# jchen8tw/ewn-gym

Measured on AMD Instinct MI355X. Metric: env steps/sec (whole node), 5x5 EWN, depth-3 expectiminimax opponent, higher is better.
Workload: dtype u32 bitboards (int8 boards in HBM), f64 expectation

## Files before the change

ewn_gym_amd/csrc/ewn_rollout.hpp:

```cpp
#pragma once
#include "ewn_step_d3.hpp"


#ifdef EWN_ROLLOUT_STAMPS
#define RSTAMP(i) do { unsigned long long t_; asm volatile("s_memtime %0\n\ts_waitcnt lgkmcnt(0)" : "=s"(t_) :: "memory"); st_acc[i] += t_ - st_prev; st_prev = t_; } while (0)
#else
#define RSTAMP(i) do { } while (0)
#endif

struct RollCfg {
    int N, autoreset, lane_offset, depth, agent_depth, K;
    int agent_sample;
    u32 seed_stride, W;
    double reward;
    u64 key;
};

struct RollBuf {
    int8_t *board; int8_t *dice; uint8_t *done; u32 *rng;
    const void *tables;
    const void *agent_tables;
    int8_t *t_board; int8_t *t_dice; int8_t *t_action; double *t_reward; uint8_t *t_term; uint8_t *t_trunc; uint8_t *t_info;
    uint8_t *t_rec;
    double *ret_sum; int32_t *n_steps; int32_t *n_episodes; int32_t *n_wins;
};

template <int S>
EWN_DEV RState<S> rs_flip(const FastTab<S> *Tb, const RState<S> &s)
{
    typedef typename MaskOf<S>::type M;
    RState<S> f;
    u32 rp[6], rn[6];
    #pragma unroll
    for (int k = 0; k < 6; k++) { rp[k] = Tb->rot[pk_get(s.posN, k) & 63]; rn[k] = Tb->rot[pk_get(s.posP, k) & 63]; }
    f.posP = PK_PADS; f.posN = PK_PADS; f.P = 0; f.N = 0;
    #pragma unroll
    for (int k = 0; k < 6; k++) {
        const bool ap = !(pk_get(s.posN, k) & PK_OFF), an = !(pk_get(s.posP, k) & PK_OFF);
        f.posP |= (u64)(ap ? rp[k] : (u32)PK_OFF) << (8 * k);
        f.posN |= (u64)(an ? rn[k] : (u32)PK_OFF) << (8 * k);
        f.P |= ap ? ((M)1 << rp[k]) : (M)0;
        f.N |= an ? ((M)1 << rn[k]) : (M)0;
    }
    return f;
}

template <int S> struct RecGeo {
    static constexpr int CELLS = S * S, STR = (CELLS + 6 + 15) & ~15, NCH = STR / 16;
    static_assert(STR == EWN_TRAJ_RECORD_STRIDE(S), "include/ewn_hip.h states the stride");
};

template <int S> struct InitRec {
    u32 w[RecGeo<S>::STR / 4];
    constexpr InitRec() : w()
    {
        int b[RecGeo<S>::STR] = {};
        int cnt = 1;
        for (int i = 1; i <= 3; i++)
            for (int j = 0; j < i; j++) { b[j * S + (i - j - 1)] = cnt; b[(S - 1 - j) * S + (S - i + j)] = -cnt; cnt++; }
        for (int i = 0; i < RecGeo<S>::STR; i++) w[i / 4] |= (u32)(b[i] & 0xFF) << (8 * (i % 4));
    }
};

template <int S, int T>
EWN_DEV void rec_slot_build(const FastTab<S> *Tb, const RState<S> &s, int sub, int8_t *slot)
{
    #pragma unroll
    for (int c0 = 0; c0 < RecGeo<S>::NCH; c0 += T) { const int c = c0 + sub; if (c < RecGeo<S>::NCH) ((uint4 *)slot)[c] = make_uint4(0u, 0u, 0u, 0u); }
    __builtin_amdgcn_wave_barrier();
    d3_encode_cubes<S, T>(Tb, s, sub, slot);
    __builtin_amdgcn_wave_barrier();
}

template <int S, int T = 1>
EWN_DEV void rec_slot_init(int8_t *slot, int sub = 0)
{
    constexpr InitRec<S> I{};
    #pragma unroll
    for (int c0 = 0; c0 < RecGeo<S>::NCH; c0 += T) {
        const int c = c0 + sub;
        u32 w[4] = { I.w[4 * c0], I.w[4 * c0 + 1], I.w[4 * c0 + 2], I.w[4 * c0 + 3] };
        #pragma unroll
        for (int cc = c0 + 1; cc < c0 + T && cc < RecGeo<S>::NCH; cc++)
            #pragma unroll
            for (int i = 0; i < 4; i++) w[i] = c == cc ? I.w[4 * cc + i] : w[i];
        if (c < RecGeo<S>::NCH) ((uint4 *)slot)[c] = make_uint4(w[0], w[1], w[2], w[3]);
    }
}

template <int S, int T>
EWN_DEV void rec_store(const int8_t *slot, int sub, int dice, int aflag, int adir, int term, int trunc, int info, uint8_t *dst)
{
    constexpr int CELLS = RecGeo<S>::CELLS, NCH = RecGeo<S>::NCH;
    const u32 meta[6] = { (u32)dice & 0xFFu, (u32)aflag & 0xFFu, (u32)adir & 0xFFu, (u32)term, (u32)trunc, (u32)info };
    #pragma unroll
    for (int c0 = 0; c0 < NCH; c0 += T) {
        const int c = c0 + sub;
        if (c < NCH) {
            const uint4 v = ((const uint4 *)slot)[c];
            u32 w[4] = { v.x, v.y, v.z, v.w };
            #pragma unroll
            for (int cc = c0; cc < c0 + T && cc < NCH; cc++) {
                u32 add[4] = { 0u, 0u, 0u, 0u };
                bool any = false;
                #pragma unroll
                for (int m = 0; m < 6; m++) {
                    const int off = CELLS + m;
                    if (off / 16 == cc) { add[(off % 16) / 4] |= meta[m] << (8 * (off % 4)); any = true; }
                }
                if (any) {
                    const bool me = T == 1 || c == cc;
                    #pragma unroll
                    for (int i = 0; i < 4; i++) w[i] |= me ? add[i] : 0u;
                }
            }
            *(uint4 *)(dst + 16 * c) = make_uint4(w[0], w[1], w[2], w[3]);
        }
    }
}


template <int S>
EWN_DEV void roll_stand_in_action(const FastTab<S> *Tb, u32 okm, u32 e, LaneRng &r, const RollCfg &c, int game, int &aflag, int &adir)
{
    const int n = __popc(okm);
    const u32 w = agent_hash(r.seed_mix(), r.draws(), (u32)(c.lane_offset + game), c.key);
    if (c.agent_sample) {
        const int a6 = (int)__umulhi(w, 6u);
        aflag = a6 >= 3 ? 1 : 0;
        adir = a6 - 3 * aflag;
    } else if (n > 0) {
        const int slot = Tb->nth[okm * 8u + __umulhi(w, (u32)n)];
        aflag = slot < 3 ? (int)(e >> 15) : 0;
        adir = slot < 3 ? slot : slot - 3;
    }
}
template <int S>
EWN_DEV void roll_stand_in_action(const FastTab<S> *Tb, const RState<S> &s, u32 e, LaneRng &r, const RollCfg &c, int game, int &aflag, int &adir)
{
    const u32 pp = pk_pair(s.posN, e);
    roll_stand_in_action<S>(Tb, (u32)Tb->lgn[pp & 0xFFu] | ((u32)Tb->lgn[pp >> 8] << 3), e, r, c, game, aflag, adir);
}

template <int S>
EWN_DEV void slot_move(const FastTab<S> *Tb, int8_t *slot, int pb, int q, int v)
{
    const int cp = Tb->real_of_ring[pb & 63], cq = Tb->real_of_ring[q & 63]; slot[cp] = 0; slot[cq] = (int8_t)v;
}

template <int S>
EWN_DEV bool roll_agent_half(const FastTab<S> *Tb, RState<S> &s, u32 e, int aflag, int adir, int &dice, LaneRng &r, double R,
                             double &reward, int &term, int &trunc, int &info, int8_t *slot = nullptr)
{
    const int k = pk_cube(e, aflag == 1);
    const int pb = pk_get(s.posN, k);
    const int q = Tb->nbn[adir][pb];
    if (q == 255) { reward = -R; term = 1; trunc = 1; info = EWN_INFO_INVALID_PLAYER; return false; }
    if (slot) slot_move<S>(Tb, slot, pb, q, k + 1);
    rs_move<S, false>(s, k, q);
    if (q == Tb->ri_origin || s.P == 0) { reward = R; term = 1; info = EWN_INFO_WON; return false; }
    dice = r.randint(1, 7);
    return true;
}

template <int S>
EWN_DEV void roll_opponent_move(const FastTab<S> *Tb, RState<S> &s, int k, int pb, int q, int &dice, LaneRng &r, double R,
                                double &reward, int &term, int &info, int8_t *slot = nullptr)
{
    if (slot) slot_move<S>(Tb, slot, pb, q, -(k + 1));
    rs_move<S, true>(s, k, q);
    if (q == FastTab<S>::CELLS - 1 || s.N == 0) { reward = -R; term = 1; info = EWN_INFO_LOST; }
    else dice = r.randint(1, 7);
}

template <int S>
EWN_DEV void roll_opponent_half(const FastTab<S> *Tb, RState<S> &s, u32 e, int oflag, int odir, int &dice, LaneRng &r, double R,
                                double &reward, int &term, int &info, int8_t *slot = nullptr)
{
    const int k = pk_cube(e, oflag == 1);
    const int pb = pk_get(s.posP, k);
    const int q = Tb->nbp[odir][pb];
    roll_opponent_move<S>(Tb, s, k, pb, q, dice, r, R, reward, term, info, slot);
}


template <int S>
EWN_DEV void roll_stand_in_action(const FastTab<S> *Tb, const MoveEnt &m0, const MoveEnt &m1, u32 e, LaneRng &r, const RollCfg &c, int game, int &aflag, int &adir)
{
    roll_stand_in_action<S>(Tb, me_legal(m0) | (me_legal(m1) << 3), e, r, c, game, aflag, adir);
}

template <int T>
EWN_DEV void slot_move_real(int8_t *slot, int sub, u32 w, int shp, int shq, int v)
{
    static_assert(T == 1 || T == 2, "one or two lanes per game");
    if constexpr (T == 1) { slot[(w >> shp) & 0xFFu] = 0; slot[(w >> shq) & 0xFFu] = (int8_t)v; }
    else {
        const bool dst = sub == 1;
        slot[(w >> (dst ? shq : shp)) & 0xFFu] = (int8_t)(dst ? v : 0);
    }
}

template <int S, int T>
EWN_DEV bool roll_agent_half(RState<S> &s, const MoveEnt &m0, const MoveEnt &m1, u32 e, int aflag, int adir, int &dice, LaneRng &r,
                             const LaneRng::StepDice *sd, double R, double &reward, int &term, int &trunc, int &info, int8_t *slot, int sub)
{
    const bool first = aflag == 1 || ((e >> 8) & 7u) == 6u;
    const int k = pk_cube(e, aflag == 1);
    MoveEnt m;
    m.mv = first ? m0.mv : m1.mv; m.rc = first ? m0.rc : m1.rc;
    const int q = me_dest(m, adir);
    if (q == 255) { reward = -R; term = 1; trunc = 1; info = EWN_INFO_INVALID_PLAYER; return false; }
    if (slot) slot_move_real<T>(slot, sub, m.rc, 0, 8 + 8 * adir, k + 1);
    rs_move<S, false>(s, k, q);
    constexpr RingGeo<S> G{};
    if (q == G.ring_of_rm[0] || s.P == 0) { reward = R; term = 1; info = EWN_INFO_WON; return false; }
    if (sd) { dice = sd->d1; r.ps.n = sd->n1; }
    else dice = r.randint(1, 7);
    return true;
}

template <int S, int T>
EWN_DEV void roll_opponent_move_real(RState<S> &s, int k, int q, u32 w, int shp, int shq, int &dice, LaneRng &r,
                                     const LaneRng::StepDice *sd, double R, double &reward, int &term, int &info, int8_t *slot, int sub)
{
    if (slot) slot_move_real<T>(slot, sub, w, shp, shq, -(k + 1));
    rs_move<S, true>(s, k, q);
    if (q == FastTab<S>::CELLS - 1 || s.N == 0) { reward = -R; term = 1; info = EWN_INFO_LOST; }
    else if (sd) { dice = sd->d2; r.ps.n = sd->n2; }
    else dice = r.randint(1, 7);
}

template <int S, int T, int OPP, int RNGK, int AGENT, bool H2 = false, int TRJ = 0>
__global__ __launch_bounds__(D3_BS, ((OPP == 2 || AGENT == 2) ? 2 : 1)) void k_rollout_d3(RollCfg c, RollBuf B)
{
    constexpr int CELLS = S * S, GPB = D3_BS / T;
    extern __shared__ __attribute__((aligned(16))) int8_t lds_dyn[];
    constexpr int LDS_STATIC = AGENT == 0 ? ((GPB * CELLS + 15) & ~15) + FAST_TAB_BYTES(S) + GPB * 16 + GPB * RecGeo<S>::STR : 16;
    __shared__ __attribute__((aligned(16))) int8_t lds_st[LDS_STATIC];
    int8_t *lds = AGENT == 0 ? lds_st : lds_dyn;
    int8_t *tb = lds + ((GPB * CELLS + 15) & ~15);
    tables_to_lds<FAST_TAB_BYTES(S)>(tb, (const int8_t *)B.tables);
    const FastTab<S> *Tb = (const FastTab<S> *)tb;
    const FastTab<S> *Ta = Tb;
    int8_t *after = tb + FAST_TAB_BYTES(S);
    if (AGENT != 0 && B.agent_tables != B.tables) {
        tables_to_lds<FAST_TAB_BYTES(S)>(after, (const int8_t *)B.agent_tables);
        Ta = (const FastTab<S> *)after;
        after += FAST_TAB_BYTES(S);
    }
    uint8_t *garr = (uint8_t *)after;
    int8_t *rec_slot = (int8_t *)garr + GPB * 16 + ((int)threadIdx.x / T) * RecGeo<S>::STR;

    const int g0 = (int)blockIdx.x * GPB, ng = min(GPB, c.N - g0);
    const int gl = threadIdx.x / T, sub = threadIdx.x % T, game = g0 + gl;
    const bool live = game < c.N, writer = live && sub == 0;

    uint4 hdr = make_uint4(0u, 0u, 0u, 0u);
    int dice = 1;
    bool frozen = true;
    if (live) {
        hdr = *rng_hdr_ptr(B.rng, game);
        dice = B.dice[game];
        frozen = B.done[game] != 0;
    }
    const bool frozen0 = frozen;
    block_copy_in(lds, B.board + (size_t)g0 * CELLS, ng * CELLS);
    LaneRng r; r.load(RNGK, hdr, rng_win_ptr(B.rng, c.N, c.W, live ? game : 0, RNGF_CUR(hdr.w)), c.W, c.key);
    r.begin_kernel();
    lds_dma_wait();
    __syncthreads();
    int8_t *mine = lds + gl * CELLS;
    RState<S> s;
    d3_decode<S, T>(live ? mine : lds, sub, garr + gl * 16, s);
    const bool want_board = TRJ == 0 && B.t_board != nullptr;
    double ret_acc = 0.0;
    int n_steps = 0, n_eps = 0, n_wins = 0;

#ifdef EWN_ROLLOUT_STAMPS
    unsigned long long st_acc[6] = { 0, 0, 0, 0, 0, 0 }, st_prev;
    asm volatile("s_memtime %0\n\ts_waitcnt lgkmcnt(0)" : "=s"(st_prev) :: "memory");
    const unsigned long long st_begin = st_prev;
#endif
    #pragma unroll 1
    for (int kstep = 0; kstep < c.K; kstep++) {
        const bool active = live && !frozen;
        double reward = 0.0;
        int term = 0, trunc = 0, info = EWN_INFO_NONE;
        if (live && frozen) term = 1;
        int aflag = 0, adir = 0;
        if constexpr (AGENT == 0) {
            roll_stand_in_action<S>(Tb, s, pk_sel<S>(Tb, s.posN, dice), r, c, game, aflag, adir);
        } else {
            const RState<S> f = rs_flip<S>(Ta, s);
            if constexpr (AGENT == 1) d3_search<S, T>(Ta, f, dice, sub, c.agent_depth, aflag, adir);
            else d5_dispatch<S, T>(Ta, f, dice, sub, aflag, adir);
        }
        if (active) {
            if constexpr (RNGK == 0) r.prefetch();
            r.begin_step();
            if constexpr (RNGK == 1) r.ps.prime();
        }
        RSTAMP(0);
        bool reply = false;
        if (active) reply = roll_agent_half<S>(Tb, s, pk_sel<S>(Tb, s.posN, dice), aflag, adir, dice, r, c.reward, reward, term, trunc, info);
        RSTAMP(1);
        int oflag = 0, odir = 0;
        if constexpr (OPP == 0) d3_search<S, T, H2>(Tb, s, dice, sub, c.depth, oflag, odir);
        if constexpr (OPP == 2) d5_dispatch<S, T, H2>(Tb, s, dice, sub, oflag, odir);
        RSTAMP(2);
        if (reply) {
            const u32 e = pk_sel<S>(Tb, s.posP, dice);
            if constexpr (OPP == 1) {
                const u32 pp = pk_pair(s.posP, e);
                const u32 okm = (u32)Tb->lgp[pp & 0xFFu] | ((u32)Tb->lgp[pp >> 8] << 3);
                const int slot = Tb->nth[okm * 8u + (u32)r.randint(0, __popc(okm))];
                oflag = slot < 3 ? (int)(e >> 15) : 0;
                odir = slot < 3 ? slot : slot - 3;
            }
            roll_opponent_half<S>(Tb, s, e, oflag, odir, dice, r, c.reward, reward, term, info);
        }
        if (active) {
            ret_acc += reward; n_steps++; n_eps += term; n_wins += info == EWN_INFO_WON ? 1 : 0;
            if (term) {
                if (c.autoreset) {
                    r.next_episode(B.rng, c.N, game, c.seed_stride, c.key, nullptr);
                    d3_init_state<S>(Tb, s);
                    dice = r.first_dice(6);
                } else frozen = true;
            }
        }
        RSTAMP(3);
        if constexpr (TRJ == 1) {
            if (writer) B.t_reward[(size_t)kstep * c.N + game] = reward;
        } else if (writer) {
            const size_t o = (size_t)kstep * c.N + game;
            if (B.t_action) ((uint16_t *)B.t_action)[o] = (uint16_t)((uint8_t)aflag | ((uint16_t)(uint8_t)adir << 8));
            if (B.t_dice) B.t_dice[o] = (int8_t)dice;
            if (B.t_reward) B.t_reward[o] = reward;
            if (B.t_term) B.t_term[o] = (uint8_t)term;
            if (B.t_trunc) B.t_trunc[o] = (uint8_t)trunc;
            if (B.t_info) B.t_info[o] = (uint8_t)info;
        }
        if (TRJ == 1 || B.t_rec) {
            rec_slot_build<S, T>(Tb, s, sub, rec_slot);
            if (live) rec_store<S, T>(rec_slot, sub, dice, aflag, adir, term, trunc, info, B.t_rec + ((size_t)kstep * c.N + game) * RecGeo<S>::STR);
            __builtin_amdgcn_wave_barrier();
        }
        if (want_board) {
            int8_t *row = B.t_board + ((size_t)kstep * c.N + g0) * CELLS;
            constexpr int WB = (64 / T) * CELLS;
            static_assert(WB % 16 == 0, "a wave's span of boards is a whole number of 16-byte pieces");
            if (ng == GPB && (((uintptr_t)row) & 15) == 0) {
                const int wv = threadIdx.x >> 6, ln = threadIdx.x & 63;
                uint4 *span = (uint4 *)(lds + wv * WB);
                __builtin_amdgcn_wave_barrier();
                #pragma unroll
                for (int i = 0; i < (WB / 16 + 63) / 64; i++) { const int j = i * 64 + ln; if (j < WB / 16) span[j] = make_uint4(0u, 0u, 0u, 0u); }
                __builtin_amdgcn_wave_barrier();
                d3_encode_cubes<S, T>(Tb, s, sub, mine);
                __builtin_amdgcn_wave_barrier();
                uint4 *dst = (uint4 *)(row + wv * WB);
                #pragma unroll
                for (int i = 0; i < (WB / 16 + 63) / 64; i++) { const int j = i * 64 + ln; if (j < WB / 16) dst[j] = span[j]; }
                __builtin_amdgcn_wave_barrier();
            } else {
                if (live) d3_encode<S, T>(Tb, s, sub, mine);
                __syncthreads();
                block_copy_out(row, lds, ng * CELLS);
                __syncthreads();
            }
        }
        RSTAMP(4);
    }
#ifdef EWN_ROLLOUT_STAMPS
    if (B.ret_sum && (threadIdx.x & 63) == 0) {
        unsigned long long *o = (unsigned long long *)B.ret_sum + (size_t)(blockIdx.x * (D3_BS / 64) + (threadIdx.x >> 6)) * 8;
        for (int i = 0; i < 6; i++) o[i] = st_acc[i];
        o[6] = st_begin; o[7] = st_prev;
    }
#endif
    if (live) d3_encode<S, T>(Tb, s, sub, mine);
    if (writer) {
        if (!frozen0) { *rng_hdr_ptr(B.rng, game) = r.header(); B.dice[game] = (int8_t)dice; }
        B.done[game] = frozen ? 1 : 0;
#ifndef EWN_ROLLOUT_STAMPS
        if (B.ret_sum) B.ret_sum[game] += ret_acc;
#endif
        if (B.n_steps) B.n_steps[game] += n_steps;
        if (B.n_episodes) B.n_episodes[game] += n_eps;
        if (B.n_wins) B.n_wins[game] += n_wins;
    }
    __syncthreads();
    block_copy_out(B.board + (size_t)g0 * CELLS, lds, ng * CELLS);
}

template <int S, int T, int OPP, int RNGK, bool H2 = false, int TRJ = 0>
__global__ __launch_bounds__(D3_BS, (OPP == 2 ? 2 : 1)) void k_rollout_slots(RollCfg c, RollBuf B)
{
    static_assert(OPP == 0 || OPP == 2, "minimax opponents");
    static_assert(!(H2 && OPP == 2), "'two_min_dist' at max_depth 5 / 6 keeps the reference's loops (d5_search): lock-step kernel only");
    constexpr int CELLS = S * S, GPB = D3_BS / T;
    constexpr int STR = RecGeo<S>::STR;
    constexpr bool PH = OPP == 0 && !H2 && slot_phantom<S>;
    __shared__ __attribute__((aligned(16))) int8_t lds_st[GPB * STR + FAST_TAB_BYTES(S) + GPB * 16 + SlotTabGeo<S, PH>::EXTRA];
    int8_t *lds = lds_st;
    int8_t *tb = lds + GPB * STR;
    tables_to_lds<FAST_TAB_BYTES(S)>(tb, (const int8_t *)B.tables);
    const FastTab<S> *Tb = (const FastTab<S> *)tb;
    uint8_t *garr = (uint8_t *)(tb + FAST_TAB_BYTES(S));
    const SlotTabs<S, PH> D = slot_tabs_at<S, PH>(tb, (int8_t *)garr + GPB * 16);

    const int g0 = (int)blockIdx.x * GPB, ng = min(GPB, c.N - g0);
    const int gl = threadIdx.x / T, sub = threadIdx.x % T, game = g0 + gl;
    const bool live = game < c.N, writer = live && sub == 0;

    uint4 hdr = make_uint4(0u, 0u, 0u, 0u);
    int dice = 1;
    bool frozen = true;
    if (live) {
        hdr = *rng_hdr_ptr(B.rng, game);
        dice = B.dice[game];
        frozen = B.done[game] != 0;
    }
    const bool frozen0 = frozen;
    block_copy_in(lds, B.board + (size_t)g0 * CELLS, ng * CELLS);
    LaneRng r; r.load(RNGK, hdr, rng_win_ptr(B.rng, c.N, c.W, live ? game : 0, RNGF_CUR(hdr.w)), c.W, c.key);
    r.begin_kernel();
    lds_dma_wait();
    __syncthreads();
    for (int e = threadIdx.x; e < 256; e += D3_BS) slot_tabs_build<S, PH>(Tb, D, e);
    RState<S> s;
    d3_decode<S, T>(live ? lds + gl * CELLS : lds, sub, garr + gl * 16, s);
    __syncthreads();
    int8_t *slot_b = lds + gl * STR;
    const bool want_slot = TRJ == 1 || (TRJ == 0 && (B.t_board != nullptr || B.t_rec != nullptr));
    int8_t *slot_m = want_slot ? slot_b : nullptr;
    if (want_slot) rec_slot_build<S, T>(Tb, s, sub, slot_b);
    double ret_acc = 0.0;
    int n_steps = 0, n_eps = 0, n_wins = 0;

    int kdone = 0, phase = 0;
    double reward = 0.0, best = 0.0;
    int term = 0, trunc = 0, info = EWN_INFO_NONE, aflag = 0, adir = 0, oflag = 0, odir = 0;
    u32 omove = 0;
    bool reply = false;
    LaneRng::StepDice sdv; sdv.d1 = sdv.d2 = 1; sdv.n1 = sdv.n2 = 0;
    const LaneRng::StepDice *sd = RNGK == 1 ? &sdv : nullptr;
    const int klim = live ? c.K : 0;
#ifdef EWN_ROLLOUT_STAMPS
    unsigned long long st_acc[6] = { 0, 0, 0, 0, 0, 0 }, st_prev;
    asm volatile("s_memtime %0\n\ts_waitcnt lgkmcnt(0)" : "=s"(st_prev) :: "memory");
    const unsigned long long st_begin = st_prev;
#endif
    while (true) {
        const bool pending = kdone < klim;
        if (__builtin_amdgcn_ballot_w64(pending) == 0) break;
        const bool start = pending && phase == 0;
        const bool active = start && !frozen;
        if (start) {
            reward = 0.0; term = frozen ? 1 : 0; trunc = 0; info = EWN_INFO_NONE; reply = false; aflag = 0; adir = 0;
            const u32 esel = pk_sel<S>(Tb, s.posN, dice);
            MoveEnt m0 = {}, m1 = {};
            const u32 pp = pk_pair(s.posN, esel);
            m0 = me_read(D.mvn, (int)(pp & 0xFFu)); m1 = me_read(D.mvn, (int)((pp >> 8) & 0xFFu));
            roll_stand_in_action<S>(Tb, m0, m1, esel, r, c, game, aflag, adir);
            if (active) {
                if constexpr (RNGK == 0) r.prefetch();
                r.begin_step();
                if constexpr (RNGK == 1) { if constexpr (T == 2) r.ps.prime_pair(sub); else r.ps.prime(); sdv = r.step_dice(); }
                reply = roll_agent_half<S, T>(s, m0, m1, esel, aflag, adir, dice, r, sd, c.reward, reward, term, trunc, info, slot_m, sub);
            }
        }
        RSTAMP(0);
        bool second = false;
        if constexpr (OPP == 0) best = d3_search<S, T, H2, true, PH>(Tb, s, dice, sub, c.depth, oflag, odir, phase, best, &second, &omove, &D);
        else best = d5c_search<S, T, true>(Tb, s, dice, sub, oflag, odir, phase, best, &second);
        RSTAMP(1);
        if (pending && phase == 0 && reply && second) phase = 1;
        else if (pending) {
            phase = 0;
            if (reply) {
                if constexpr (OPP == 0) {
                    roll_opponent_move_real<S, T>(s, (int)(omove & 7u), (int)((omove >> 8) & 0xFFu), omove, 16, 24, dice, r, sd, c.reward, reward, term, info, slot_m, sub);
                } else {
                    const int k = pk_cube(pk_sel<S>(Tb, s.posP, dice), oflag == 1), pb = pk_get(s.posP, k);
                    const MoveEnt mp = me_read(D.mvp, pb);
                    roll_opponent_move_real<S, T>(s, k, me_dest(mp, odir), mp.rc, 0, 8 + 8 * odir, dice, r, sd, c.reward, reward, term, info, slot_m, sub);
                }
            }
            if (!frozen) {
                ret_acc += reward; n_steps++; n_eps += term; n_wins += info == EWN_INFO_WON ? 1 : 0;
                if (term) {
                    if (c.autoreset) {
                        r.next_episode(B.rng, c.N, game, c.seed_stride, c.key, nullptr);
                        d3_init_state<S>(Tb, s);
                        if (want_slot) rec_slot_init<S, T>(slot_b, sub);
                        dice = r.first_dice(6);
                    } else frozen = true;
                }
            }
            RSTAMP(2);
            const size_t o = (size_t)kdone * c.N + game;
            if constexpr (TRJ == 1) {
                if (sub == 0) B.t_reward[o] = reward;
            } else if (TRJ == 0 && sub == 0) {
                if (B.t_action) ((uint16_t *)B.t_action)[o] = (uint16_t)((uint8_t)aflag | ((uint16_t)(uint8_t)adir << 8));
                if (B.t_dice) B.t_dice[o] = (int8_t)dice;
                if (B.t_reward) B.t_reward[o] = reward;
                if (B.t_term) B.t_term[o] = (uint8_t)term;
                if (B.t_trunc) B.t_trunc[o] = (uint8_t)trunc;
                if (B.t_info) B.t_info[o] = (uint8_t)info;
            }
            if (want_slot) __builtin_amdgcn_wave_barrier();
            if (TRJ == 1 || (TRJ == 0 && B.t_rec)) rec_store<S, T>(slot_b, sub, dice, aflag, adir, term, trunc, info, B.t_rec + o * STR);
            if (TRJ == 0 && B.t_board) {
                constexpr int CH = ((CELLS / T + 3) & ~3) < CELLS ? ((CELLS / T + 3) & ~3) : (CELLS & ~3);
                int8_t *dst = B.t_board + o * CELLS;
                #pragma unroll
                for (int i = 0; i < CH; i += 4) {
                    const int at = sub * CH + i;
                    if (at + 4 <= CELLS) { const u32 w = *(const u32 *)(slot_b + at); __builtin_memcpy(dst + at, &w, 4); }
                }
                if (sub == T - 1) {
                    #pragma unroll
                    for (int i = (T * CH < CELLS ? T * CH : (CELLS & ~3)); i < CELLS; i++) dst[i] = slot_b[i];
                }
            }
            kdone++;
        }
        RSTAMP(3);
#ifdef EWN_ROLLOUT_STAMPS
        st_acc[4]++;
#endif
    }
#ifdef EWN_ROLLOUT_STAMPS
    if (B.ret_sum && (threadIdx.x & 63) == 0) {
        unsigned long long *o = (unsigned long long *)B.ret_sum + (size_t)(blockIdx.x * (D3_BS / 64) + (threadIdx.x >> 6)) * 8;
        for (int i = 0; i < 6; i++) o[i] = st_acc[i];
        o[6] = st_begin; o[7] = st_prev;
    }
#endif
    __syncthreads();
    if (live) d3_encode<S, T>(Tb, s, sub, lds + gl * CELLS);
    if (writer) {
        if (!frozen0) { *rng_hdr_ptr(B.rng, game) = r.header(); B.dice[game] = (int8_t)dice; }
        B.done[game] = frozen ? 1 : 0;
#ifndef EWN_ROLLOUT_STAMPS
        if (B.ret_sum) B.ret_sum[game] += ret_acc;
#endif
        if (B.n_steps) B.n_steps[game] += n_steps;
        if (B.n_episodes) B.n_episodes[game] += n_eps;
        if (B.n_wins) B.n_wins[game] += n_wins;
    }
    __syncthreads();
    block_copy_out(B.board + (size_t)g0 * CELLS, lds, ng * CELLS);
}
```

ewn_gym_amd/csrc/ewn_step_d3.hpp:

```cpp
#pragma once
#include "ewn_fast.hpp"
#include "ewn_movetab.hpp"

template <int S>
struct RingGeo {
    int ring_of_rm[S * S];
    int rm_of_ring[S * S];
    constexpr RingGeo() : ring_of_rm(), rm_of_ring()
    {
        int n = 0;
        for (int t = 0; t < S; t++)
            for (int i = 0; i < S; i++)
                for (int j = 0; j < S; j++)
                    if ((i < j ? i : j) == t) { ring_of_rm[i * S + j] = n; rm_of_ring[n] = i * S + j; n++; }
    }
};

template <int CTRL> EWN_DEV u32 dpp_u32(u32 v) { return (u32)__builtin_amdgcn_update_dpp(0, (int)v, CTRL, 0xF, 0xF, true); }
template <int CTRL> EWN_DEV double dpp_f64(double v)
{
    const u64 b = (u64)__double_as_longlong(v);
    const u32 lo = dpp_u32<CTRL>((u32)b), hi = dpp_u32<CTRL>((u32)(b >> 32));
    return __longlong_as_double((long long)(((u64)hi << 32) | lo));
}
template <int T, int J> struct Bcast {
    static_assert(T == 2, "pairs (0,1) and (2,3) of a quad");
    static constexpr int CTRL = J | (J << 2) | ((2 + J) << 4) | ((2 + J) << 6);
};
#define DPP_XOR1 0xB1

EWN_DEV int pk_get(u64 w, int k) { return (int)((w >> (8 * k)) & 0xFFull); }
#define PK_OFF 0x40
#define PK_PADS (0x4040ull << 48)

template <int S>
struct RState {
    typename MaskOf<S>::type P, N;
    u64 posP, posN;
};

EWN_DEV u32 pk_alive(u64 w)
{
    const u32 t = (~(u32)w & 0x40404040u) >> 6, u = ~(u32)(w >> 32);
    return ((t | (t >> 7) | (t >> 14) | (t >> 21)) & 0xFu) | ((u >> 2) & 0x10u) | ((u >> 9) & 0x20u);
}

template <int S>
EWN_DEV u32 pk_sel(const FastTab<S> *Tb, u64 pos, int dice) { return Tb->sel[pk_alive(pos) * 8u + ((u32)(dice - 1) & 7u)]; }
EWN_DEV u32 pk_pair(u64 pos, u32 e) { return __builtin_amdgcn_perm((u32)(pos >> 32), (u32)pos, (e & 0x0707u) | 0x0C0C0000u); }
EWN_DEV int pk_cube(u32 e, bool larger) { const int first = (int)(e & 7u), second = (int)((e >> 8) & 7u); return (larger || second == 6) ? first : second; }

EWN_DEV u64 pk_capture(u64 w, u32 qb)
{
    u32 lo = (u32)w, hi = (u32)(w >> 32);
    lo |= (((lo ^ qb) + 0x01010101u) >> 1) & 0x40404040u;
    hi |= (((hi ^ qb) + 0x01010101u) >> 1) & 0x40404040u;
    return ((u64)hi << 32) | lo;
}

template <int S, bool MOVER_IS_P>
EWN_DEV void rs_move(RState<S> &s, int k, int q)
{
    typedef typename MaskOf<S>::type M;
    const M one = 1, bq = one << q;
    const int p = pk_get(MOVER_IS_P ? s.posP : s.posN, k) & 63;
    const u32 q7 = (u32)q ^ 0x7Fu, qb = __builtin_amdgcn_perm(q7, q7, 0u);
    s.posP = pk_capture(s.posP, qb);
    s.posN = pk_capture(s.posN, qb);
    const u64 mv = (u64)(u32)(p ^ q) << (8 * k);
    if (MOVER_IS_P) { s.posP ^= mv; s.P = (s.P & ~(one << p)) | bq; s.N &= ~bq; }
    else { s.posN ^= mv; s.N = (s.N & ~(one << p)) | bq; s.P &= ~bq; }
}

template <int S, int T = 1, bool H2 = false>
__device__ __forceinline__ double d5_search(const FastTab<S> *Tb, const RState<S> &c, int dice, int sub, int &bflag, int &bdir)
{
    static_assert(T == 1 || T == 2, "the six dice of the inner chance node are split over one or two lanes");
    typedef typename MaskOf<S>::type M;
    const M one = 1;
    const double inf = __builtin_inf();
    u32 rank10 = 8u * (u32)Tb->nv;
    while (ft_val<S>(Tb, rank10) > 10.0) rank10 -= 8u;
    double best = -inf, alpha = -inf;
    bflag = 0; bdir = 0;
    const u32 e0 = pk_sel<S>(Tb, c.posP, dice), pp0 = pk_pair(c.posP, e0);
    #pragma unroll 1
    for (int r = 0; r < 6; r++) {
        const int slot = r >= 3 ? 1 : 0, dir = r - 3 * slot;
        const int cube = (int)((slot ? e0 >> 8 : e0) & 7u), rb = (int)((slot ? pp0 >> 8 : pp0) & 0xFFu);
        const int dest = Tb->nbp[dir][rb];
        if (dest == 255) continue;
        RState<S> s1 = c;
        rs_move<S, true>(s1, cube, dest);
        double v;
        if (dest == FastTab<S>::CELLS - 1 || s1.N == 0) v = 10.0;
        else {
            v = 0.0;
            #pragma unroll 1
            for (int d1 = 1; d1 <= 6; d1++) {
                const u32 e1 = pk_sel<S>(Tb, s1.posN, d1), pp1 = pk_pair(s1.posN, e1);
                double worst = inf, beta = inf;
                #pragma unroll 1
                for (int q = 0; q < 6; q++) {
                    const int qs = q >= 3 ? 1 : 0, qd = q - 3 * qs;
                    const int qc = (int)((qs ? e1 >> 8 : e1) & 7u), qb = (int)((qs ? pp1 >> 8 : pp1) & 0xFFu);
                    const int dn = Tb->nbn[qd][qb];
                    if (dn == 255) continue;
                    RState<S> s2 = s1;
                    rs_move<S, false>(s2, qc, dn);
                    double val;
                    if (dn == Tb->ri_origin || s2.P == 0) val = -10.0;
                    else {
                        val = 0.0;
                        u32 br[6 / T];
                        #pragma unroll
                        for (int j = 0; j < 6 / T; j++) {
                            const int d2 = sub + 1 + T * j;
                            const u32 e2 = pk_sel<S>(Tb, s2.posP, d2), pp2 = pk_pair(s2.posP, e2);
                            u32 lx[6], ly[6], lr[6];
                            bool ex[6], won[6];
                            #pragma unroll
                            for (int m = 0; m < 6; m++) {
                                const int ms = m >= 3 ? 1 : 0, md = m - 3 * ms;
                                const int mb = (int)((ms ? pp2 >> 8 : pp2) & 0xFFu);
                                const int dp = Tb->nbp[md][mb];
                                ex[m] = dp != 255;
                                const M bd = ex[m] ? (one << (dp & 63)) : (M)0;
                                const M P3 = (s2.P & ~(one << (mb & 63))) | bd, N3 = s2.N & ~bd;
                                won[m] = dp == FastTab<S>::CELLS - 1 || N3 == 0;
                                lx[m] = ft_side_h<S, H2>(Tb, P3);
                                ly[m] = ft_side_h<S, H2>(Tb, N3);
                            }
                            __builtin_amdgcn_sched_barrier(0);
                            #pragma unroll
                            for (int m = 0; m < 6; m++) lr[m] = ft_rank8<S>(Tb, ft_addr(lx[m], ly[m]));
                            __builtin_amdgcn_sched_barrier(0);
                            double lv[6];
                            #pragma unroll
                            for (int m = 0; m < 6; m++) { lr[m] = won[m] ? rank10 : lr[m]; lv[m] = ft_val<S>(Tb, lr[m]); }
                            __builtin_amdgcn_sched_barrier(0);
                            u32 bestr = 0;
                            double bestv = -inf;
                            bool stop = false;
                            #pragma unroll
                            for (int m = 0; m < 6; m++) {
                                const bool live = ex[m] && !stop;
                                bestr = live ? max(bestr, lr[m]) : bestr;
                                bestv = live ? fmax(bestv, lv[m]) : bestv;
                                stop = stop || (live && beta <= fmax(alpha, bestv));
                            }
                            br[j] = bestr;
                        }
                        u32 bd6[6];
                        #pragma unroll
                        for (int j = 0; j < 6 / T; j++) {
                            if constexpr (T == 1) bd6[j] = br[j];
                            else { bd6[2 * j] = dpp_u32<Bcast<2, 0>::CTRL>(br[j]); bd6[2 * j + 1] = dpp_u32<Bcast<2, 1>::CTRL>(br[j]); }
                        }
                        double q6[6];
                        #pragma unroll
                        for (int d = 0; d < 6; d++) q6[d] = ft_val6<S>(Tb, bd6[d]);
                        #pragma unroll
                        for (int d = 0; d < 6; d++) val = val + q6[d];
                    }
                    if (val < worst) worst = val;
                    beta = fmin(beta, worst);
                    if (beta <= alpha) break;
                }
                v = v + worst / 6.0;
            }
        }
        if (v > best) { best = v; bflag = slot == 0 ? (int)(e0 >> 15) : 0; bdir = dir; }
        alpha = fmax(alpha, best);
    }
    return best;
}

#define D3_PRIO_HI() __builtin_amdgcn_s_setprio(2)
#define D3_PRIO_LO() __builtin_amdgcn_s_setprio(0)
#define D3_STAGE_FENCE() __builtin_amdgcn_sched_barrier(0)
#define D3_SEARCH_FENCE() do { if constexpr (!PERLANE) __builtin_amdgcn_sched_barrier(0); } while (0)
EWN_DEV u32 rank_u32(u32 r) { asm("" : "+v"(r)); return r; }
#define D3_CUT 0x4000u

template <int T> EWN_DEV u32 own_of(const u32 (&v)[6], int i, int sub)
{
    static_assert(T == 1 || T == 2, "one or two lanes per game");
    if constexpr (T == 1) return v[i];
    else return sub ? v[2 * i + 1] : v[2 * i];
}

template <int T> EWN_DEV void publish(u32 mine, int i, u32 (&out)[6])
{
    static_assert(T == 1 || T == 2, "one or two lanes per game");
    if constexpr (T == 1) out[i] = mine;
    else { out[2 * i] = dpp_u32<Bcast<2, 0>::CTRL>(mine); out[2 * i + 1] = dpp_u32<Bcast<2, 1>::CTRL>(mine); }
}

template <int S, int T, bool H2 = false, bool PERLANE = false, bool PH = false>
__device__ __forceinline__ double d3_search(const FastTab<S> *Tb, const RState<S> &c, int dice, int sub, int depth, int &bflag, int &bdir,
                                            int slotL = 0, double best_in = 0.0, bool *have_second = nullptr, u32 *bmove = nullptr,
                                            [[maybe_unused]] const SlotTabs<S, PH> *D = nullptr)
{
    static_assert(T == 1 || T == 2, "the six replier cubes and dice values are split over one or two lanes");
    static_assert(!PH || (PERLANE && !H2 && slot_phantom<S>), "phantom cells: the slot-task form on 5x5 and 6x6, (level, count) images");
    typedef typename MaskOf<S>::type M;
    constexpr int KPT = 6 / T;
    const M one = 1;
    constexpr bool PAIR = PERLANE && T == 2;

    const u32 rsel_all = pk_sel<S>(Tb, c.posP, dice), rpp_all = pk_pair(c.posP, rsel_all);
    const u32 rsel = PERLANE ? rsel_all >> (8 * slotL) : rsel_all, rpp = PERLANE ? rpp_all >> (8 * slotL) : rpp_all;
    const int rb0 = (int)(rpp & 0xFFu), rb1 = (int)(rpp >> 8);
    const bool have0 = !(rb0 & PK_OFF), have1 = !(rb1 & PK_OFF);
    const int flag0 = (int)(rsel >> 15);
    const int rp0 = rb0 & 63, rp1 = rb1 & 63;
    [[maybe_unused]] const u32 rc0 = rsel & 7u, rc1 = (rsel >> 8) & 7u;
    u32 bm = 0;
    [[maybe_unused]] MoveEnt me0 = {};
    [[maybe_unused]] u32 rm0 = 0;
    if constexpr (PERLANE) {
        me0 = me_read(D->mvp, rb0);
        rm0 = (me0.mv & 0xFFFFFF00u) | rc0;
    }
    #define D3_BM_SEL(d) (0x05040100u + (u32)(d) * 0x01000100u)

    double best = -__builtin_inf();
    if constexpr (PERLANE) {
        *have_second = !(rpp_all & ((u32)PK_OFF << 8));
        if (slotL == 0) { bflag = 0; bdir = 0; } else best = best_in;
        if (bmove && slotL != 0) bm = *bmove;
    } else { bflag = 0; bdir = 0; }

    if (depth < 3) {
        [[maybe_unused]] MoveEnt me1 = {};
        if constexpr (PERLANE) { me1 = me_read(D->mvp, rb1); me1.mv = (me1.mv & 0xFFFFFF00u) | rc1; }
        #pragma unroll 1
        for (int r = 0; r < 6; r++) {
            const int slot = r >= 3 ? 1 : 0, dir = r - 3 * slot;
            const int rp = slot == 0 ? rp0 : rp1;
            int dest;
            [[maybe_unused]] const u32 rcw = slot == 0 ? me0.rc : me1.rc, mvw = slot == 0 ? rm0 : me1.mv;
            if constexpr (PERLANE) dest = (int)((mvw >> (8 + 8 * dir)) & 0xFFu); else dest = Tb->nbp[dir][rp];
            const bool valid = (slot == 0 ? have0 : have1) && dest != 255;
            const M bd = valid ? (one << dest) : (M)0;
            const M P1 = (c.P & ~(one << rp)) | bd;
            const M N1 = c.N & ~bd;
            const bool term = dest == FastTab<S>::CELLS - 1 || N1 == 0;
            const u32 rk = ft_rank8<S>(Tb, ft_addr(ft_side_h<S, H2>(Tb, P1), ft_side_h<S, H2>(Tb, N1)));
            const double e1 = ft_val<S>(Tb, rk), e6 = ft_val6<S>(Tb, rk);
            double v = 0.0;
            #pragma unroll
            for (int d = 0; d < 6; d++) v = v + e6;
            v = term ? 10.0 : (depth == 1 ? e1 : v);
            if (valid && v > best) {
                best = v; bflag = slot == 0 ? flag0 : 0; bdir = dir;
                if constexpr (PERLANE) bm = __builtin_amdgcn_perm(rcw, mvw, D3_BM_SEL(dir));
            }
        }
        if constexpr (PERLANE) { *have_second = false; if (bmove) *bmove = bm; }
        return best;
    }

    M rset[KPT][3], rclr[KPT];
    int rnk[KPT];
    [[maybe_unused]] u32 keep[KPT][3], fixed[KPT][3];
    #pragma unroll
    for (int i = 0; i < KPT; i++) {
        const int k = sub + T * i;
        const int rb = pk_get(c.posN, k);
        rnk[i] = rb & 63;
        rclr[i] = ~(one << rnk[i]);
        if constexpr (PH) {
            typedef u32 u32x4 __attribute__((ext_vector_type(4)));
            typedef __attribute__((address_space(3))) const volatile u32x4 lds_u4;
            lds_u4 *re = (lds_u4 *)(D->rep + rb);
            if constexpr (sizeof(M) == 4) {
                const u32x4 a = re[0];
                rset[i][0] = a.x; rset[i][1] = a.y; rset[i][2] = a.z;
            } else {
                const u32x4 a = re[0], b = re[1];
                rset[i][0] = ((u64)a.y << 32) | a.x; rset[i][1] = ((u64)a.w << 32) | a.z; rset[i][2] = ((u64)b.y << 32) | b.x;
            }
        } else if constexpr (PERLANE) {
            const ReplyEnt<S> *re = D->rep + rb;
            u32 kf[3];
            if constexpr (sizeof(M) == 4) {
                const uint4 a = *(const uint4 *)re; const uint2 b = *((const uint2 *)re + 2);
                rset[i][0] = a.x; rset[i][1] = a.y; rset[i][2] = a.z; kf[0] = a.w; kf[1] = b.x; kf[2] = b.y;
            } else {
                const uint4 a = *(const uint4 *)re, b = *((const uint4 *)re + 1); const u32 t = *((const u32 *)re + 8);
                rset[i][0] = ((u64)a.y << 32) | a.x; rset[i][1] = ((u64)a.w << 32) | a.z; rset[i][2] = ((u64)b.y << 32) | b.x;
                kf[0] = b.z; kf[1] = b.w; kf[2] = t;
            }
            #pragma unroll
            for (int d = 0; d < 3; d++) { keep[i][d] = kf[d]; fixed[i][d] = kf[d] >> 16; }
        } else {
        #pragma unroll
        for (int d = 0; d < 3; d++) {
            const u32 kf = Tb->rkf[d][rb];
            rset[i][d] = Tb->rsetT[d][rb];
            keep[i][d] = kf;
            fixed[i][d] = kf >> 16;
        }
        }
    }

    u32 dq0;
    if constexpr (PERLANE) dq0 = me0.mv >> 8;
    else dq0 = (u32)Tb->nbp[0][rp0] | ((u32)Tb->nbp[1][rp0] << 8) | ((u32)Tb->nbp[2][rp0] << 16);
    [[maybe_unused]] u32 dq1 = 0;
    if constexpr (!PERLANE) dq1 = (u32)Tb->nbp[0][rp1] | ((u32)Tb->nbp[1][rp1] << 8) | ((u32)Tb->nbp[2][rp1] << 16);

    constexpr int ROOT_UNROLL = PERLANE ? 3 : 1;
    D3_PRIO_HI();
    #pragma unroll ROOT_UNROLL
    for (int r = 0; r < (PERLANE ? 3 : 6); r++) {
        const int slot = PERLANE ? 0 : (r >= 3 ? 1 : 0), dir = PERLANE ? r : r - 3 * slot;
        const int rp = slot == 0 ? rp0 : rp1;
        const int dest = (int)(((slot == 0 ? dq0 : dq1) >> (8 * dir)) & 0xFFu);
        const bool valid = PERLANE ? dest != 255 : ((slot == 0 ? have0 : have1) && dest != 255);
        const M bd = valid ? (one << dest) : (M)0;
        const M P1 = (c.P & ~(one << rp)) | bd;
        const M N1 = c.N & ~bd;
        const bool term = dest == FastTab<S>::CELLS - 1 || N1 == 0;

        [[maybe_unused]] u32 tr[6];
        [[maybe_unused]] u32 km[KPT];
        constexpr int CH = 3;
        #pragma unroll
        for (int i0 = 0; i0 < KPT; i0 += CH) {
            M P2[CH][3], N2[CH][3];
            u32 lp[CH][3], ln[CH][3], a[CH][3];
            #pragma unroll
            for (int ii = 0; ii < CH; ii++) {
                const M Nk = N1 & rclr[i0 + ii];
                #pragma unroll
                for (int d = 0; d < 3; d++) {
                    N2[ii][d] = Nk | rset[i0 + ii][d];
                    P2[ii][d] = P1 & ~rset[i0 + ii][d];
                    lp[ii][d] = Tb->lvl[lvl_index(P2[ii][d])];
                    ln[ii][d] = Tb->lvl[lvl_index(N2[ii][d])];
                    if constexpr (H2) {
                        lp[ii][d] += Tb->lvl[lvl_index(drop_top(P2[ii][d]))];
                        ln[ii][d] += Tb->lvl[lvl_index(drop_top(N2[ii][d]))];
                    }
                }
            }
            D3_SEARCH_FENCE();
            #pragma unroll
            for (int ii = 0; ii < CH; ii++) {
                #pragma unroll
                for (int d = 0; d < 3; d++) {
                    const u32 ix = H2 ? lp[ii][d] : lp[ii][d] + (u32)popc_m(P2[ii][d]), iy = H2 ? ln[ii][d] : ln[ii][d] + (u32)popc_m(N2[ii][d]);
                    if constexpr (PH) a[ii][d] = rank_u32(ft_rank8<S>(Tb, ft_addr(ix, iy)));
                    else a[ii][d] = rank_u32(ft_rank8<S>(Tb, (ft_addr(ix, iy) & keep[i0 + ii][d]) | fixed[i0 + ii][d]));
                }
            }
            D3_SEARCH_FENCE();
            u32 p1[CH], p2[CH];
            double va[CH], v1[CH], v2[CH];
            #pragma unroll
            for (int ii = 0; ii < CH; ii++) {
                p1[ii] = min(a[ii][0], a[ii][1]); p2[ii] = min(p1[ii], a[ii][2]);
// ... 446 lines not shown
```

Measured before the change: 13.88 billion.

## Pack step metadata into record words and compute selector index with udot4

After: 13.84 billion (median of 3 runs). Within noise of the previous version (-0.3%).

```diff
diff --git a/ewn_gym_amd/csrc/ewn_rollout.hpp b/ewn_gym_amd/csrc/ewn_rollout.hpp
--- a/ewn_gym_amd/csrc/ewn_rollout.hpp
+++ b/ewn_gym_amd/csrc/ewn_rollout.hpp
@@ -119,6 +119,40 @@
     }
 }
 
+enum { META_DICE = 0, META_AFLAG, META_ADIR, META_TERM, META_TRUNC, META_INFO };
+template <int S> struct MetaGeo {
+    static constexpr int CELLS = S * S, PIECE = CELLS / 16, W0 = (CELLS % 16) / 4;
+    static constexpr int word(int m) { return ((CELLS + m) % 16) / 4 - W0; }
+    static constexpr int sh(int m) { return 8 * ((CELLS + m) % 4); }
+    static_assert((CELLS + 5) / 16 == PIECE && ((CELLS + 5) % 16) / 4 - W0 <= 1, "six meta bytes: one piece, two words");
+};
+template <int S, int M> EWN_DEV void meta_or(u32 (&w)[2], u32 v) { w[MetaGeo<S>::word(M)] |= v << MetaGeo<S>::sh(M); }
+template <int S, int M> EWN_DEV u32 meta_get(const u32 (&w)[2]) { return (w[MetaGeo<S>::word(M)] >> MetaGeo<S>::sh(M)) & 0xFFu; }
+template <int S> EWN_DEV void meta_outcome(u32 (&w)[2], u32 term, u32 trunc, u32 info)
+{
+    meta_or<S, META_TERM>(w, term); meta_or<S, META_TRUNC>(w, trunc); meta_or<S, META_INFO>(w, info);
+}
+
+template <int S, int T>
+EWN_DEV void rec_store_packed(const int8_t *slot, int sub, u32 own, u32 ma, u32 mb, uint8_t *dst)
+{
+    typedef u32 u32x4 __attribute__((ext_vector_type(4)));
+    constexpr int NCH = RecGeo<S>::NCH, PIECE = MetaGeo<S>::PIECE, W0 = MetaGeo<S>::W0;
+    #pragma unroll
+    for (int c0 = 0; c0 < NCH; c0 += T) {
+        const int c = c0 + sub;
+        if (c < NCH) {
+            u32x4 v = ((const u32x4 *)slot)[c];
+            if (c0 <= PIECE && PIECE < c0 + T) {
+                u32x4 add = { 0u, 0u, 0u, 0u };
+                add[W0] = T == 1 ? ma : (ma & own); add[W0 + 1] = T == 1 ? mb : (mb & own);
+                v |= add;
+            }
+            *(u32x4 *)(dst + 16 * c0) = v;
+        }
+    }
+}
+
 
 template <int S>
 EWN_DEV void roll_stand_in_action(const FastTab<S> *Tb, u32 okm, u32 e, LaneRng &r, const RollCfg &c, int game, int &aflag, int &adir)
@@ -203,18 +237,18 @@
 
 template <int S, int T>
 EWN_DEV bool roll_agent_half(RState<S> &s, const MoveEnt &m0, const MoveEnt &m1, u32 e, int aflag, int adir, int &dice, LaneRng &r,
-                             const LaneRng::StepDice *sd, double R, double &reward, int &term, int &trunc, int &info, int8_t *slot, int sub)
+                             const LaneRng::StepDice *sd, double R, double &reward, u32 (&mw)[2], int &n_eps, int &n_wins, int8_t *slot, int sub)
 {
     const bool first = aflag == 1 || ((e >> 8) & 7u) == 6u;
     const int k = pk_cube(e, aflag == 1);
     MoveEnt m;
     m.mv = first ? m0.mv : m1.mv; m.rc = first ? m0.rc : m1.rc;
     const int q = me_dest(m, adir);
-    if (q == 255) { reward = -R; term = 1; trunc = 1; info = EWN_INFO_INVALID_PLAYER; return false; }
+    if (q == 255) { reward = -R; meta_outcome<S>(mw, 1u, 1u, EWN_INFO_INVALID_PLAYER); n_eps++; return false; }
     if (slot) slot_move_real<T>(slot, sub, m.rc, 0, 8 + 8 * adir, k + 1);
     rs_move<S, false>(s, k, q);
     constexpr RingGeo<S> G{};
-    if (q == G.ring_of_rm[0] || s.P == 0) { reward = R; term = 1; info = EWN_INFO_WON; return false; }
+    if (q == G.ring_of_rm[0] || s.P == 0) { reward = R; meta_outcome<S>(mw, 1u, 0u, EWN_INFO_WON); n_eps++; n_wins++; return false; }
     if (sd) { dice = sd->d1; r.ps.n = sd->n1; }
     else dice = r.randint(1, 7);
     return true;
@@ -222,11 +256,11 @@
 
 template <int S, int T>
 EWN_DEV void roll_opponent_move_real(RState<S> &s, int k, int q, u32 w, int shp, int shq, int &dice, LaneRng &r,
-                                     const LaneRng::StepDice *sd, double R, double &reward, int &term, int &info, int8_t *slot, int sub)
+                                     const LaneRng::StepDice *sd, double R, double &reward, u32 (&mw)[2], int &n_eps, int8_t *slot, int sub)
 {
     if (slot) slot_move_real<T>(slot, sub, w, shp, shq, -(k + 1));
     rs_move<S, true>(s, k, q);
-    if (q == FastTab<S>::CELLS - 1 || s.N == 0) { reward = -R; term = 1; info = EWN_INFO_LOST; }
+    if (q == FastTab<S>::CELLS - 1 || s.N == 0) { reward = -R; meta_outcome<S>(mw, 1u, 0u, EWN_INFO_LOST); n_eps++; }
     else if (sd) { dice = sd->d2; r.ps.n = sd->n2; }
     else dice = r.randint(1, 7);
 }
@@ -439,10 +473,19 @@
     if (want_slot) rec_slot_build<S, T>(Tb, s, sub, slot_b);
     double ret_acc = 0.0;
     int n_steps = 0, n_eps = 0, n_wins = 0;
+    double *acc_ret = B.ret_sum; int32_t *acc_steps = B.n_steps, *acc_eps = B.n_episodes, *acc_wins = B.n_wins;
+    int8_t *st_board = B.board, *st_dice = B.dice;
+    asm("" : "+s"(acc_ret), "+s"(acc_steps), "+s"(acc_eps), "+s"(acc_wins), "+s"(st_board), "+s"(st_dice));
 
     int kdone = 0, phase = 0;
     double reward = 0.0, best = 0.0;
-    int term = 0, trunc = 0, info = EWN_INFO_NONE, aflag = 0, adir = 0, oflag = 0, odir = 0;
+    int aflag = 0, adir = 0, oflag = 0, odir = 0;
+    u32 mw[2] = { 0u, 0u };
+    u32 own = (T == 1 || sub == MetaGeo<S>::PIECE % T) ? ~0u : 0u;
+    if constexpr (T != 1) asm("" : "+v"(own));
+    const size_t rec_step = (size_t)c.N * STR;
+    uint8_t *rec_p = TRJ == 1 ? B.t_rec + (size_t)(live ? game : 0) * STR + 16 * sub : nullptr;
+    double *rew_p = TRJ == 1 ? B.t_reward + (live ? game : 0) : nullptr;
     u32 omove = 0;
     bool reply = false;
     LaneRng::StepDice sdv; sdv.d1 = sdv.d2 = 1; sdv.n1 = sdv.n2 = 0;
@@ -459,17 +502,19 @@
         const bool start = pending && phase == 0;
         const bool active = start && !frozen;
         if (start) {
-            reward = 0.0; term = frozen ? 1 : 0; trunc = 0; info = EWN_INFO_NONE; reply = false; aflag = 0; adir = 0;
-            const u32 esel = pk_sel<S>(Tb, s.posN, dice);
+            reward = 0.0; reply = false; aflag = 0; adir = 0;
+            mw[0] = mw[1] = 0u; meta_or<S, META_TERM>(mw, frozen ? 1u : 0u);
+            const u32 esel = pk_sel_dot<S>(Tb, s.posN, dice);
             MoveEnt m0 = {}, m1 = {};
             const u32 pp = pk_pair(s.posN, esel);
             m0 = me_read(D.mvn, (int)(pp & 0xFFu)); m1 = me_read(D.mvn, (int)((pp >> 8) & 0xFFu));
             roll_stand_in_action<S>(Tb, m0, m1, esel, r, c, game, aflag, adir);
+            meta_or<S, META_AFLAG>(mw, (u32)aflag); meta_or<S, META_ADIR>(mw, (u32)adir);
             if (active) {
                 if constexpr (RNGK == 0) r.prefetch();
                 r.begin_step();
                 if constexpr (RNGK == 1) { if constexpr (T == 2) r.ps.prime_pair(sub); else r.ps.prime(); sdv = r.step_dice(); }
-                reply = roll_agent_half<S, T>(s, m0, m1, esel, aflag, adir, dice, r, sd, c.reward, reward, term, trunc, info, slot_m, sub);
+                reply = roll_agent_half<S, T>(s, m0, m1, esel, aflag, adir, dice, r, sd, c.reward, reward, mw, n_eps, n_wins, slot_m, sub);
             }
         }
         RSTAMP(0);
@@ -482,16 +527,16 @@
             phase = 0;
             if (reply) {
                 if constexpr (OPP == 0) {
-                    roll_opponent_move_real<S, T>(s, (int)(omove & 7u), (int)((omove >> 8) & 0xFFu), omove, 16, 24, dice, r, sd, c.reward, reward, term, info, slot_m, sub);
+                    roll_opponent_move_real<S, T>(s, (int)(omove & 7u), (int)((omove >> 8) & 0xFFu), omove, 16, 24, dice, r, sd, c.reward, reward, mw, n_eps, slot_m, sub);
                 } else {
-                    const int k = pk_cube(pk_sel<S>(Tb, s.posP, dice), oflag == 1), pb = pk_get(s.posP, k);
+                    const int k = pk_cube(pk_sel_dot<S>(Tb, s.posP, dice), oflag == 1), pb = pk_get(s.posP, k);
                     const MoveEnt mp = me_read(D.mvp, pb);
-                    roll_opponent_move_real<S, T>(s, k, me_dest(mp, odir), mp.rc, 0, 8 + 8 * odir, dice, r, sd, c.reward, reward, term, info, slot_m, sub);
+                    roll_opponent_move_real<S, T>(s, k, me_dest(mp, odir), mp.rc, 0, 8 + 8 * odir, dice, r, sd, c.reward, reward, mw, n_eps, slot_m, sub);
                 }
             }
             if (!frozen) {
-                ret_acc += reward; n_steps++; n_eps += term; n_wins += info == EWN_INFO_WON ? 1 : 0;
-                if (term) {
+                ret_acc += reward; n_steps++;
+                if (meta_get<S, META_TERM>(mw)) {
                     if (c.autoreset) {
                         r.next_episode(B.rng, c.N, game, c.seed_stride, c.key, nullptr);
                         d3_init_state<S>(Tb, s);
@@ -501,19 +546,25 @@
                 }
             }
             RSTAMP(2);
-            const size_t o = (size_t)kdone * c.N + game;
+            const size_t o = TRJ == 0 ? (size_t)kdone * c.N + game : 0;
+            const u32 mwd = mw[MetaGeo<S>::word(META_DICE)] | ((u32)dice << MetaGeo<S>::sh(META_DICE));
+            const u32 ma = MetaGeo<S>::word(META_DICE) == 0 ? mwd : mw[0], mb = mw[1];
             if constexpr (TRJ == 1) {
-                if (sub == 0) B.t_reward[o] = reward;
+                if (sub == 0) *rew_p = reward;
             } else if (TRJ == 0 && sub == 0) {
-                if (B.t_action) ((uint16_t *)B.t_action)[o] = (uint16_t)((uint8_t)aflag | ((uint16_t)(uint8_t)adir << 8));
+                const u32 mc[2] = { ma, mb };
+                if (B.t_action) ((uint16_t *)B.t_action)[o] = (uint16_t)(meta_get<S, META_AFLAG>(mc) | (meta_get<S, META_ADIR>(mc) << 8));
                 if (B.t_dice) B.t_dice[o] = (int8_t)dice;
                 if (B.t_reward) B.t_reward[o] = reward;
-                if (B.t_term) B.t_term[o] = (uint8_t)term;
-                if (B.t_trunc) B.t_trunc[o] = (uint8_t)trunc;
-                if (B.t_info) B.t_info[o] = (uint8_t)info;
+                if (B.t_term) B.t_term[o] = (uint8_t)meta_get<S, META_TERM>(mc);
+                if (B.t_trunc) B.t_trunc[o] = (uint8_t)meta_get<S, META_TRUNC>(mc);
+                if (B.t_info) B.t_info[o] = (uint8_t)meta_get<S, META_INFO>(mc);
             }
             if (want_slot) __builtin_amdgcn_wave_barrier();
-            if (TRJ == 1 || (TRJ == 0 && B.t_rec)) rec_store<S, T>(slot_b, sub, dice, aflag, adir, term, trunc, info, B.t_rec + o * STR);
+            if constexpr (TRJ == 1) {
+                rec_store_packed<S, T>(slot_b, sub, own, ma, mb, rec_p);
+                rec_p += rec_step; rew_p += c.N;
+            } else if (TRJ == 0 && B.t_rec) rec_store_packed<S, T>(slot_b, sub, own, ma, mb, B.t_rec + o * STR + 16 * sub);
             if (TRJ == 0 && B.t_board) {
                 constexpr int CH = ((CELLS / T + 3) & ~3) < CELLS ? ((CELLS / T + 3) & ~3) : (CELLS & ~3);
                 int8_t *dst = B.t_board + o * CELLS;
@@ -544,15 +595,15 @@
     __syncthreads();
     if (live) d3_encode<S, T>(Tb, s, sub, lds + gl * CELLS);
     if (writer) {
-        if (!frozen0) { *rng_hdr_ptr(B.rng, game) = r.header(); B.dice[game] = (int8_t)dice; }
+        if (!frozen0) { *rng_hdr_ptr(B.rng, game) = r.header(); st_dice[game] = (int8_t)dice; }
         B.done[game] = frozen ? 1 : 0;
 #ifndef EWN_ROLLOUT_STAMPS
-        if (B.ret_sum) B.ret_sum[game] += ret_acc;
-#endif
-        if (B.n_steps) B.n_steps[game] += n_steps;
-        if (B.n_episodes) B.n_episodes[game] += n_eps;
-        if (B.n_wins) B.n_wins[game] += n_wins;
+        if (acc_ret) acc_ret[game] += ret_acc;
+#endif
+        if (acc_steps) acc_steps[game] += n_steps;
+        if (acc_eps) acc_eps[game] += n_eps;
+        if (acc_wins) acc_wins[game] += n_wins;
     }
     __syncthreads();
-    block_copy_out(B.board + (size_t)g0 * CELLS, lds, ng * CELLS);
-}
+    block_copy_out(st_board + (size_t)g0 * CELLS, lds, ng * CELLS);
+}
diff --git a/ewn_gym_amd/csrc/ewn_step_d3.hpp b/ewn_gym_amd/csrc/ewn_step_d3.hpp
--- a/ewn_gym_amd/csrc/ewn_step_d3.hpp
+++ b/ewn_gym_amd/csrc/ewn_step_d3.hpp
@@ -47,6 +47,19 @@
 
 template <int S>
 EWN_DEV u32 pk_sel(const FastTab<S> *Tb, u64 pos, int dice) { return Tb->sel[pk_alive(pos) * 8u + ((u32)(dice - 1) & 7u)]; }
+__host__ EWN_DEV u32 pk_sel_index(u64 w, int dice)
+{
+    const u32 l6 = (u32)w >> 6, h2 = (u32)(w >> 32) >> 2;
+    const u32 off = (l6 & 0x01010101u) | (h2 & ~0x01010101u);
+    const u32 on = ~off & 0x01011111u, d = (u32)(dice - 1) & 7u;
+#if defined(__HIP_DEVICE_COMPILE__)
+    return __builtin_amdgcn_udot4(on, 0x40201008u, d, false);
+#else
+    return d + 8u * (on & 0xFFu) + 16u * ((on >> 8) & 0xFFu) + 32u * ((on >> 16) & 0xFFu) + 64u * (on >> 24);
+#endif
+}
+template <int S>
+EWN_DEV u32 pk_sel_dot(const FastTab<S> *Tb, u64 pos, int dice) { return Tb->sel[pk_sel_index(pos, dice)]; }
 EWN_DEV u32 pk_pair(u64 pos, u32 e) { return __builtin_amdgcn_perm((u32)(pos >> 32), (u32)pos, (e & 0x0707u) | 0x0C0C0000u); }
 EWN_DEV int pk_cube(u32 e, bool larger) { const int first = (int)(e & 7u), second = (int)((e >> 8) & 7u); return (larger || second == 6) ? first : second; }
 
@@ -209,7 +222,7 @@
     const M one = 1;
     constexpr bool PAIR = PERLANE && T == 2;
 
-    const u32 rsel_all = pk_sel<S>(Tb, c.posP, dice), rpp_all = pk_pair(c.posP, rsel_all);
+    const u32 rsel_all = PERLANE ? pk_sel_dot<S>(Tb, c.posP, dice) : pk_sel<S>(Tb, c.posP, dice), rpp_all = pk_pair(c.posP, rsel_all);
     const u32 rsel = PERLANE ? rsel_all >> (8 * slotL) : rsel_all, rpp = PERLANE ? rpp_all >> (8 * slotL) : rpp_all;
     const int rb0 = (int)(rpp & 0xFFu), rb1 = (int)(rpp >> 8);
     const bool have0 = !(rb0 & PK_OFF), have1 = !(rb1 & PK_OFF);
```
